# asd56585452/IGS

Hardware: AMD Instinct MI355X
Metric: Gaussians rendered/sec (fwd+bwd) at 1352x1014; PSNR vs ref (higher is better)
Workload: dtype f32; 1 GPU; BASELINE.json configs[2]: sear_steak-like frame-0 stand-in, 200000 Gaussians, SH degree 3, 10 train cams @1352x1014; per step and rank one view: fwd + L1 loss + bwd + Adam; scene=bench, points=200000, width=1352, height=1014, views=10, loss=l1, clamp=False, parallelism=one GPU: the whole step inside igs_refine_step, no exchange

## Files before the change

igs_amd/csrc/geom_bwd.hip:

```cpp
#include "geom_math.h"
#include "../../include/igs_rast.h"

__constant__ float BSH_C0 = 0.28209479177387814f;
__constant__ float BSH_C1 = 0.4886025119029199f;
__constant__ float BSH_C2[5] = { 1.0925484305920792f, -1.0925484305920792f, 0.31539156525252005f, -1.0925484305920792f,
                                 0.5462742152960396f };
__constant__ float BSH_C3[7] = { -0.5900435899266435f, 2.890611442640554f, -0.4570457994644658f, 0.3731763325901154f,
                                 -0.4570457994644658f, 1.445305721320277f, -0.5900435899266435f };

__device__ __forceinline__ float3 dnormvdv(float3 v, float3 dv) {
    const float sum2 = v.x * v.x + v.y * v.y + v.z * v.z;
    const float invsum32 = 1.0f / sqrtf(sum2 * sum2 * sum2);
    float3 r;
    r.x = ((+sum2 - v.x * v.x) * dv.x - v.y * v.x * dv.y - v.z * v.x * dv.z) * invsum32;
    r.y = (-v.x * v.y * dv.x + (sum2 - v.y * v.y) * dv.y - v.z * v.y * dv.z) * invsum32;
    r.z = (-v.x * v.z * dv.x - v.y * v.z * dv.y + (sum2 - v.z * v.z) * dv.z) * invsum32;
    return r;
}

__device__ __forceinline__ float3 sh_backward(int deg, int M, const float* __restrict__ sh, float3 dir_orig, uint32_t clamped,
                                              float3 dL_dcolor, float* __restrict__ dsh)
{
    const float len = sqrtf(dot3(dir_orig, dir_orig));
    const float x = dir_orig.x / len, y = dir_orig.y / len, z = dir_orig.z / len;
    const float3 g = make_float3((clamped & 1u) ? 0.f : dL_dcolor.x, (clamped & 2u) ? 0.f : dL_dcolor.y, (clamped & 4u) ? 0.f : dL_dcolor.z);
    auto L = [&](int k) { return make_float3(sh[3 * k], sh[3 * k + 1], sh[3 * k + 2]); };
    auto W = [&](int k, float b) { dsh[3 * k] = b * g.x; dsh[3 * k + 1] = b * g.y; dsh[3 * k + 2] = b * g.z; };
    float3 dx = make_float3(0, 0, 0), dy = make_float3(0, 0, 0), dz = make_float3(0, 0, 0);
    W(0, BSH_C0);
    if (deg > 0) {
        W(1, -BSH_C1 * y); W(2, BSH_C1 * z); W(3, -BSH_C1 * x);
        dx = L(3) * (-BSH_C1); dy = L(1) * (-BSH_C1); dz = L(2) * BSH_C1;
        if (deg > 1) {
            const float xx = x * x, yy = y * y, zz = z * z, xy = x * y, yz = y * z, xz = x * z;
            W(4, BSH_C2[0] * xy); W(5, BSH_C2[1] * yz); W(6, BSH_C2[2] * (2.f * zz - xx - yy)); W(7, BSH_C2[3] * xz);
            W(8, BSH_C2[4] * (xx - yy));
            dx = dx + (L(4) * (BSH_C2[0] * y) + L(6) * (BSH_C2[2] * 2.f * -x) + L(7) * (BSH_C2[3] * z) + L(8) * (BSH_C2[4] * 2.f * x));
            dy = dy + (L(4) * (BSH_C2[0] * x) + L(5) * (BSH_C2[1] * z) + L(6) * (BSH_C2[2] * 2.f * -y) + L(8) * (BSH_C2[4] * 2.f * -y));
            dz = dz + (L(5) * (BSH_C2[1] * y) + L(6) * (BSH_C2[2] * 2.f * 2.f * z) + L(7) * (BSH_C2[3] * x));
            if (deg > 2) {
                W(9, BSH_C3[0] * y * (3.f * xx - yy)); W(10, BSH_C3[1] * xy * z); W(11, BSH_C3[2] * y * (4.f * zz - xx - yy));
                W(12, BSH_C3[3] * z * (2.f * zz - 3.f * xx - 3.f * yy)); W(13, BSH_C3[4] * x * (4.f * zz - xx - yy));
                W(14, BSH_C3[5] * z * (xx - yy)); W(15, BSH_C3[6] * x * (xx - 3.f * yy));
                dx = dx + (L(9) * (BSH_C3[0] * 3.f * 2.f * xy) + L(10) * (BSH_C3[1] * yz) + L(11) * (BSH_C3[2] * -2.f * xy)
                           + L(12) * (BSH_C3[3] * -3.f * 2.f * xz) + L(13) * (BSH_C3[4] * (-3.f * xx + 4.f * zz - yy))
                           + L(14) * (BSH_C3[5] * 2.f * xz) + L(15) * (BSH_C3[6] * 3.f * (xx - yy)));
                dy = dy + (L(9) * (BSH_C3[0] * 3.f * (xx - yy)) + L(10) * (BSH_C3[1] * xz)
                           + L(11) * (BSH_C3[2] * (-3.f * yy + 4.f * zz - xx)) + L(12) * (BSH_C3[3] * -3.f * 2.f * yz)
                           + L(13) * (BSH_C3[4] * -2.f * xy) + L(14) * (BSH_C3[5] * -2.f * yz) + L(15) * (BSH_C3[6] * -3.f * 2.f * xy));
                dz = dz + (L(10) * (BSH_C3[1] * xy) + L(11) * (BSH_C3[2] * 4.f * 2.f * yz) + L(12) * (BSH_C3[3] * 3.f * (2.f * zz - xx - yy))
                           + L(13) * (BSH_C3[4] * 4.f * 2.f * xz) + L(14) * (BSH_C3[5] * (xx - yy)));
            }
        }
    }
    const int used = (deg + 1) * (deg + 1);
    for (int k = used; k < M; k++) { dsh[3 * k] = 0.f; dsh[3 * k + 1] = 0.f; dsh[3 * k + 2] = 0.f; }
    const float3 dL_ddir = make_float3(dot3(dx, g), dot3(dy, g), dot3(dz, g));
    return dnormvdv(dir_orig, dL_ddir);
}

__device__ __forceinline__ float3 sh_backward_dir_only(int deg, const float* __restrict__ sh, float3 dir_orig, uint32_t clamped, float3 dL_dcolor)
{
    const float len = sqrtf(dot3(dir_orig, dir_orig));
    const float x = dir_orig.x / len, y = dir_orig.y / len, z = dir_orig.z / len;
    const float3 g = make_float3((clamped & 1u) ? 0.f : dL_dcolor.x, (clamped & 2u) ? 0.f : dL_dcolor.y, (clamped & 4u) ? 0.f : dL_dcolor.z);
    auto L = [&](int k) { return make_float3(sh[3 * k], sh[3 * k + 1], sh[3 * k + 2]); };
    float3 dx = make_float3(0, 0, 0), dy = make_float3(0, 0, 0), dz = make_float3(0, 0, 0);
    if (deg > 0) {
        dx = L(3) * (-BSH_C1); dy = L(1) * (-BSH_C1); dz = L(2) * BSH_C1;
        if (deg > 1) {
            const float xx = x * x, yy = y * y, zz = z * z, xy = x * y, yz = y * z, xz = x * z;
            dx = dx + (L(4) * (BSH_C2[0] * y) + L(6) * (BSH_C2[2] * 2.f * -x) + L(7) * (BSH_C2[3] * z) + L(8) * (BSH_C2[4] * 2.f * x));
            dy = dy + (L(4) * (BSH_C2[0] * x) + L(5) * (BSH_C2[1] * z) + L(6) * (BSH_C2[2] * 2.f * -y) + L(8) * (BSH_C2[4] * 2.f * -y));
            dz = dz + (L(5) * (BSH_C2[1] * y) + L(6) * (BSH_C2[2] * 2.f * 2.f * z) + L(7) * (BSH_C2[3] * x));
            if (deg > 2) {
                dx = dx + (L(9) * (BSH_C3[0] * 3.f * 2.f * xy) + L(10) * (BSH_C3[1] * yz) + L(11) * (BSH_C3[2] * -2.f * xy)
                           + L(12) * (BSH_C3[3] * -3.f * 2.f * xz) + L(13) * (BSH_C3[4] * (-3.f * xx + 4.f * zz - yy))
                           + L(14) * (BSH_C3[5] * 2.f * xz) + L(15) * (BSH_C3[6] * 3.f * (xx - yy)));
                dy = dy + (L(9) * (BSH_C3[0] * 3.f * (xx - yy)) + L(10) * (BSH_C3[1] * xz)
                           + L(11) * (BSH_C3[2] * (-3.f * yy + 4.f * zz - xx)) + L(12) * (BSH_C3[3] * -3.f * 2.f * yz)
                           + L(13) * (BSH_C3[4] * -2.f * xy) + L(14) * (BSH_C3[5] * -2.f * yz) + L(15) * (BSH_C3[6] * -3.f * 2.f * xy));
                dz = dz + (L(10) * (BSH_C3[1] * xy) + L(11) * (BSH_C3[2] * 4.f * 2.f * yz) + L(12) * (BSH_C3[3] * 3.f * (2.f * zz - xx - yy))
                           + L(13) * (BSH_C3[4] * 4.f * 2.f * xz) + L(14) * (BSH_C3[5] * (xx - yy)));
            }
        }
    }
    const float3 dL_ddir = make_float3(dot3(dx, g), dot3(dy, g), dot3(dz, g));
    return dnormvdv(dir_orig, dL_ddir);
}

struct ShViewCams { float pos[3 * IGS_MAX_EXCHANGE_VIEWS]; };
struct ShAdam { float *param, *exp_avg, *exp_avg_sq; float lr_over_bc1, b1, b2, eps, inv_sqrt_bc2;
                float *sm_param = nullptr, *sm_exp_avg = nullptr, *sm_exp_avg_sq = nullptr; const float* sm_grad = nullptr;
                size_t sm_off[4] = {0, 0, 0, 0}; float sm_lr_over_bc1[4] = {0, 0, 0, 0}; };
template <bool ADAM>
__global__ void __launch_bounds__(128)
sh_grad_views_kernel(int P, int D, int M, int V, const float* __restrict__ means3D, const ShViewCams cams,
                     const float* __restrict__ gc, float clamp, float* __restrict__ dsh_out, const ShAdam ad)
{
    const float* campos = cams.pos;
    const int idx = blockIdx.x * 128 + threadIdx.x;
    const bool live = idx < P;
    if (!ADAM && !live) return;
    float acc[48];
#pragma unroll
    for (int k = 0; k < 48; k++) acc[k] = 0.f;
    const size_t ci = live ? (size_t)idx : 0;
    const float3 mean = make_float3(means3D[3 * ci], means3D[3 * ci + 1], means3D[3 * ci + 2]);
    for (int v = 0; v < (live ? V : 0); v++) {
        const float* gp = gc + ((size_t)v * P + idx) * 3;
        const float3 g = make_float3(gp[0], gp[1], gp[2]);
        if (g.x == 0.f && g.y == 0.f && g.z == 0.f) continue;
// ... 76 lines not shown
            for (int gk = 0; gk < 4; gk++) {
                const size_t o = ad.sm_off[gk] + (size_t)idx * KS[gk];
#pragma unroll
                for (int c = 0; c < KS[gk]; c++) {
                    float pp = ad.sm_param[o + c], mm = ad.sm_exp_avg[o + c], vv = ad.sm_exp_avg_sq[o + c];
                    adam_update(pp, mm, vv, ad.sm_grad[o + c], ad.sm_lr_over_bc1[gk], ad.b1, ad.b2, ad.eps, ad.inv_sqrt_bc2);
                    ad.sm_param[o + c] = pp; ad.sm_exp_avg[o + c] = mm; ad.sm_exp_avg_sq[o + c] = vv;
                }
            }
        }
        return;
    }
    float* dst = dsh_out + (size_t)idx * M * 3;
    if (M == 16 && (((uintptr_t)dsh_out) & 15) == 0) {
#pragma unroll
        for (int k = 0; k < 12; k++) ((float4*)dst)[k] = make_float4(acc[4 * k], acc[4 * k + 1], acc[4 * k + 2], acc[4 * k + 3]);
        return;
    }
#pragma unroll
    for (int k = 0; k < 16; k++)
        if (k < M) { dst[3 * k] = acc[3 * k]; dst[3 * k + 1] = acc[3 * k + 1]; dst[3 * k + 2] = acc[3 * k + 2]; }
}

hipError_t launch_sh_grad_views(hipStream_t s, int P, int D, int M, int V, const float* means3D, const float* campos_host, const float* gc,
                                float clamp, float* dsh_out)
{
    ShViewCams cams;
    for (int i = 0; i < 3 * V; i++) cams.pos[i] = campos_host[i];
    hipLaunchKernelGGL(sh_grad_views_kernel<false>, dim3((P + 127) / 128), dim3(128), 0, s, P, D, M, V, means3D, cams, gc, clamp, dsh_out, ShAdam());
    return hipGetLastError();
}

hipError_t launch_sh_adam_views(hipStream_t s, int P, int D, int M, int V, const float* means3D, const float* campos_host, const float* gc,
                                float clamp, float* param_sh, float* exp_avg_sh, float* exp_avg_sq_sh, float lr_over_bc1, float b1, float b2,
                                float eps, float inv_sqrt_bc2, const SmallGroupsAdam* sm)
{
    ShViewCams cams;
    for (int i = 0; i < 3 * V; i++) cams.pos[i] = campos_host[i];
    ShAdam ad; ad.param = param_sh; ad.exp_avg = exp_avg_sh; ad.exp_avg_sq = exp_avg_sq_sh;
    ad.lr_over_bc1 = lr_over_bc1; ad.b1 = b1; ad.b2 = b2; ad.eps = eps; ad.inv_sqrt_bc2 = inv_sqrt_bc2;
    if (sm) {
        ad.sm_param = sm->param; ad.sm_exp_avg = sm->exp_avg; ad.sm_exp_avg_sq = sm->exp_avg_sq; ad.sm_grad = sm->grad;
        for (int k = 0; k < 4; k++) { ad.sm_off[k] = sm->off[k]; ad.sm_lr_over_bc1[k] = sm->lr_over_bc1[k]; }
    }
    hipLaunchKernelGGL(sh_grad_views_kernel<true>, dim3((P + 127) / 128), dim3(128), 0, s, P, D, M, V, means3D, cams, gc, clamp, (float*)nullptr, ad);
    return hipGetLastError();
}

struct GBArgs { GeomBwdArgs a; RefineFuse f; };

#ifndef GEOM_WAVES_PER_EU
#define GEOM_WAVES_PER_EU 2
#endif
#ifdef GEOM_TIMELINE
#define GEOM_TL_MARKS 8
#define GEOM_TL_WGS 8192
__device__ unsigned long long g_geom_tl[GEOM_TL_WGS * GEOM_TL_MARKS];
extern "C" int igs_debug_geom_timeline(unsigned long long* host, int n)
{
    return (int)hipMemcpyFromSymbol(host, HIP_SYMBOL(g_geom_tl), (size_t)n * 8);
}
#define GTL(k) do { if (threadIdx.x == 0 && blockIdx.x < GEOM_TL_WGS) g_geom_tl[blockIdx.x * GEOM_TL_MARKS + (k)] = wall_clock64(); } while (0)
#else
#define GTL(k) do { } while (0)
#endif
template <bool FUSED, int NT, bool COLOUR_ONLY, bool PARTIAL = false>
__global__ void __launch_bounds__(NT) __attribute__((amdgpu_waves_per_eu(GEOM_WAVES_PER_EU)))
geom_bwd_kernel(const GBArgs args)
{
    const GeomBwdArgs& a = args.a;
    const RefineFuse& fz = args.f;
    if constexpr (FUSED) {
        if ((fz.guard_overflow && *fz.guard_overflow) || (fz.guard_prefilter && *fz.guard_prefilter)) return;
        if (blockIdx.x == 0 && threadIdx.x < 64 && fz.loss_out) {
            float v = fz.loss_scale * fz.loss_shards[16 * threadIdx.x];
            if (fz.loss_shards2) v += fz.loss_scale2 * fz.loss_shards2[16 * threadIdx.x];
            if (fz.loss_shards3) v += fz.loss_scale3 * fz.loss_shards3[16 * threadIdx.x];
#pragma unroll
            for (int off = 32; off > 0; off >>= 1) v += __shfl_down(v, off, 64);
            if (threadIdx.x == 0) fz.loss_out[0] = fz.loss_bias + v;
        }
    }
    GTL(0);
    const int ngroups = (a.P + NT - 1) / NT;
    for (int grp = blockIdx.x; grp < ngroups; grp += gridDim.x) {
    const int idx = grp * NT + threadIdx.x;
    extern __shared__ __attribute__((aligned(16))) float dsh_lds[];
    const int F = 3 * a.M, FS = F + 1;
    const bool active = idx < a.P;

    float3 o_m2d = make_float3(0, 0, 0), o_color = make_float3(0, 0, 0), o_mean = make_float3(0, 0, 0), o_scale = make_float3(0, 0, 0);
    float o_opacity = 0.f, o_cov[6] = { 0, 0, 0, 0, 0, 0 };
    float4 o_rot = make_float4(0, 0, 0, 0);
    const bool sh_frozen = PARTIAL && FUSED && (fz.frozen_groups & IGS_GROUP_SH) != 0u;
    float* dsh = (a.M && !sh_frozen) ? dsh_lds + threadIdx.x * FS : nullptr;
    bool sh_written = false;
    bool found_nan = false;
    __shared__ float small_lds[FUSED ? NT * 12 : 1];

    if (active && a.radii[idx] > 0) {
        const float4* R4 = (const float4*)(a.rec + (size_t)idx * REC_F);
        const double2* G2 = (const double2*)(a.gacc + (size_t)idx * ((COLOUR_ONLY || a.gacc_compact) ? GACC_COMPACT_F : GACC_F));
        auto G4 = [&](int k) { const double2 u = G2[2 * k], v = G2[2 * k + 1]; return make_float4((float)u.x, (float)u.y, (float)v.x, (float)v.y); };
        const float4 r0 = R4[0], r1 = R4[1], r2 = R4[2], r4 = R4[4], r5 = R4[5], r6 = R4[6], r7 = R4[7];
        PlaneCacheEntry pce; pce.have = false;
        if (!COLOUR_ONLY && a.plane_cache) pce = plane_cache_fetch(a.plane_cache + (size_t)idx * PLANE_CACHE_F);
        float4 g0, g1, g2, g3, g4, g5, g6;
        if (COLOUR_ONLY || a.gacc_compact) {
            const float4 c0 = G4(0), c1 = G4(1), c2 = G4(2);
            const float4 z = make_float4(0.f, 0.f, 0.f, 0.f);
            g0 = make_float4(c0.x, c0.y, c0.z, 0.f); g1 = z; g2 = z; g3 = z;
            g4 = make_float4(0.f, 0.f, c0.w, c1.x); g5 = make_float4(c1.y, c1.z, c1.w, c2.x); g6 = make_float4(c2.y, 0.f, 0.f, 0.f);
        } else {
            g0 = G4(0); g1 = G4(1); g2 = G4(2); g3 = G4(3); g4 = G4(4); g5 = G4(5); g6 = G4(6);
        }
        GTL(1);
        o_color = make_float3(g0.x, g0.y, g0.z);
        const float Sv0 = g0.w, Sv1 = g1.x, Sv2 = g1.y;
        const float Sx0 = g1.z, Sx1 = g1.w, Sx2 = g2.x, Sy0 = g2.y, Sy1 = g2.z, Sy2 = g2.w;
        const float St = g3.x, Stx = g3.y, Sty = g3.z;
        const float3 dL_dnormal = make_float3(g3.w, g4.x, g4.y);
        const float Q0 = g4.z, Qx = g4.w, Qy = g5.x, Qxx = g5.y, Qxy = g5.z, Qyy = g5.w, Z = g6.x;
        const float conx = r0.z, cony = r0.w, conz = r1.x, opac = r1.y;
        const float cpl[6] = { r4.x, r4.y, r4.z, r4.w, r5.x, r5.y };
        const float rplx = r2.z, rply = r2.w;
        const float halfW = 0.5f * a.W, halfH = 0.5f * a.H;
        o_m2d.x = (-(conx * Qx + cony * Qy) + cpl[0] * Sv0 + cpl[2] * Sv1 + cpl[4] * Sv2 + rplx * St) * halfW;
        o_m2d.y = (-(conz * Qy + cony * Qx) + cpl[1] * Sv0 + cpl[3] * Sv1 + cpl[5] * Sv2 + rply * St) * halfH;
        o_m2d.z = Z;
        const float dLc_x = -0.5f * Qxx, dLc_y = -0.5f * Qxy, dLc_z = -0.5f * Qyy;
        const float c0x = Sx0 / a.fx, c0y = Sy0 / a.fy, c1x = Sx1 / a.fx, c1y = Sy1 / a.fy, c2x = Sx2 / a.fx, c2y = Sy2 / a.fy;
        const float drx = Stx / a.fx, dry = Sty / a.fy;
        const float dL_dts = St;
        float dL_dopacity = (opac != 0.f) ? Q0 / opac : 0.f;

        const float3 mean = make_float3(a.means3D[3 * idx], a.means3D[3 * idx + 1], a.means3D[3 * idx + 2]);
        float cov3D[6];
        if (a.cov3D_precomp) {
#pragma unroll
            for (int k = 0; k < 6; k++) cov3D[k] = a.cov3D_precomp[6 * (size_t)idx + k];
        } else { cov3D[0] = r6.x; cov3D[1] = r6.y; cov3D[2] = r6.z; cov3D[3] = r6.w; cov3D[4] = r7.x; cov3D[5] = r7.y; }
        const uint32_t clamped = __float_as_uint(r7.z);

        const bool need_planes = !COLOUR_ONLY && ((Sv0 != 0.f) | (Sv1 != 0.f) | (Sv2 != 0.f) | (Sx0 != 0.f) | (Sx1 != 0.f) | (Sx2 != 0.f)
                                 | (Sy0 != 0.f) | (Sy1 != 0.f) | (Sy2 != 0.f) | (St != 0.f) | (Stx != 0.f) | (Sty != 0.f)
                                 | (dL_dnormal.x != 0.f) | (dL_dnormal.y != 0.f) | (dL_dnormal.z != 0.f));
        Cov2DCtx c;
        cov2d_ctx(c, mean, cov3D, a.view, a.fx, a.fy, a.tan_fovx, a.tan_fovy, a.kernel_size, need_planes,
// ... 196 lines not shown
                }
            }
        }
        if (a.scales) {
            float3 sc = make_float3(a.scales[3 * idx], a.scales[3 * idx + 1], a.scales[3 * idx + 2]);
            float4 qr = make_float4(a.rotations[4 * idx], a.rotations[4 * idx + 1], a.rotations[4 * idx + 2], a.rotations[4 * idx + 3]);
            if constexpr (FUSED) {
                sc = make_float3(act_exp(sc.x), act_exp(sc.y), act_exp(sc.z));
                const float inv = act_inv_norm4(qr.x, qr.y, qr.z, qr.w);
                qr = make_float4(qr.x * inv, qr.y * inv, qr.z * inv, qr.w * inv);
            }
            const float r = qr.x, x = qr.y, y = qr.z, z = qr.w;
            const M3 Rq = quat_rot(qr);
            const float s[3] = { a.scale_modifier * sc.x, a.scale_modifier * sc.y, a.scale_modifier * sc.z };
            float dS[3][3];
            dS[0][0] = o_cov[0]; dS[0][1] = 0.5f * o_cov[1]; dS[0][2] = 0.5f * o_cov[2];
            dS[1][0] = 0.5f * o_cov[1]; dS[1][1] = o_cov[3]; dS[1][2] = 0.5f * o_cov[4];
            dS[2][0] = 0.5f * o_cov[2]; dS[2][1] = 0.5f * o_cov[4]; dS[2][2] = o_cov[5];
            float dM[3][3];
#pragma unroll
            for (int k = 0; k < 3; k++)
#pragma unroll
                for (int b = 0; b < 3; b++)
                    dM[k][b] = (2.0f * (s[k] * Rq.m[0][k])) * dS[0][b] + (2.0f * (s[k] * Rq.m[1][k])) * dS[1][b] + (2.0f * (s[k] * Rq.m[2][k])) * dS[2][b];
            const float ds0 = Rq.m[0][0] * dM[0][0] + Rq.m[1][0] * dM[0][1] + Rq.m[2][0] * dM[0][2];
            const float ds1 = Rq.m[0][1] * dM[1][0] + Rq.m[1][1] * dM[1][1] + Rq.m[2][1] * dM[1][2];
            const float ds2 = Rq.m[0][2] * dM[2][0] + Rq.m[1][2] * dM[2][1] + Rq.m[2][2] * dM[2][2];
            o_scale = make_float3(ds0, ds1, ds2);
#define X_(a_, b_) (dM[a_][b_] * s[a_])
            o_rot.x = 2 * z * (X_(0, 1) - X_(1, 0)) + 2 * y * (X_(2, 0) - X_(0, 2)) + 2 * x * (X_(1, 2) - X_(2, 1));
            o_rot.y = 2 * y * (X_(1, 0) + X_(0, 1)) + 2 * z * (X_(2, 0) + X_(0, 2)) + 2 * r * (X_(1, 2) - X_(2, 1)) - 4 * x * (X_(2, 2) + X_(1, 1));
            o_rot.z = 2 * x * (X_(1, 0) + X_(0, 1)) + 2 * r * (X_(2, 0) - X_(0, 2)) + 2 * z * (X_(1, 2) + X_(2, 1)) - 4 * y * (X_(2, 2) + X_(0, 0));
            o_rot.w = 2 * r * (X_(0, 1) - X_(1, 0)) + 2 * x * (X_(2, 0) + X_(0, 2)) + 2 * y * (X_(1, 2) + X_(2, 1)) - 4 * z * (X_(1, 1) + X_(0, 0));
#undef X_
        }
    }
    if constexpr (FUSED) {
        if (active && fz.color_out && !sh_written) {
            fz.color_out[3 * (size_t)idx] = 0.f; fz.color_out[3 * (size_t)idx + 1] = 0.f; fz.color_out[3 * (size_t)idx + 2] = 0.f;
        }
    }
    if (active) {
        if (!FUSED || a.dL_dmean2D) {
            a.dL_dmean2D[3 * idx] = o_m2d.x; a.dL_dmean2D[3 * idx + 1] = o_m2d.y; a.dL_dmean2D[3 * idx + 2] = o_m2d.z;
        }
        if constexpr (!FUSED) {
            if (a.clamp > 0.f) {
                const float c = a.clamp;
                auto cl = [c](float x) { return x < -c ? -c : (x > c ? c : x); };
                o_mean = make_float3(cl(o_mean.x), cl(o_mean.y), cl(o_mean.z));
                o_opacity = cl(o_opacity);
                o_scale = make_float3(cl(o_scale.x), cl(o_scale.y), cl(o_scale.z));
                o_rot = make_float4(cl(o_rot.x), cl(o_rot.y), cl(o_rot.z), cl(o_rot.w));
                if (dsh && sh_written) for (int k = 0; k < F; k++) dsh[k] = cl(dsh[k]);
            }
            a.dL_dcolor[3 * idx] = o_color.x; a.dL_dcolor[3 * idx + 1] = o_color.y; a.dL_dcolor[3 * idx + 2] = o_color.z;
            a.dL_dopacity[idx] = o_opacity;
            a.dL_dmean3D[3 * idx] = o_mean.x; a.dL_dmean3D[3 * idx + 1] = o_mean.y; a.dL_dmean3D[3 * idx + 2] = o_mean.z;
#pragma unroll
            for (int k = 0; k < 6; k++) a.dL_dcov3D[6 * (size_t)idx + k] = o_cov[k];
            a.dL_dscale[3 * idx] = o_scale.x; a.dL_dscale[3 * idx + 1] = o_scale.y; a.dL_dscale[3 * idx + 2] = o_scale.z;
            a.dL_drot[4 * idx] = o_rot.x; a.dL_drot[4 * idx + 1] = o_rot.y; a.dL_drot[4 * idx + 2] = o_rot.z; a.dL_drot[4 * idx + 3] = o_rot.w;
            if (a.nan_host) {
                const float chk[17] = { o_m2d.x, o_m2d.y, o_m2d.z, o_color.x, o_color.y, o_color.z, o_opacity, o_mean.x, o_mean.y, o_mean.z,
                                        o_scale.x, o_scale.y, o_scale.z, o_rot.x, o_rot.y, o_rot.z, o_rot.w };
#pragma unroll
                for (int k = 0; k < 17; k++) found_nan |= chk[k] != chk[k];
            }
        } else {
            if (fz.clamp > 0.f) {
                const float c = fz.clamp;
                auto cl = [c](float x) { return x < -c ? -c : (x > c ? c : x); };
                o_mean = make_float3(cl(o_mean.x), cl(o_mean.y), cl(o_mean.z));
                o_opacity = cl(o_opacity);
                o_scale = make_float3(cl(o_scale.x), cl(o_scale.y), cl(o_scale.z));
                o_rot = make_float4(cl(o_rot.x), cl(o_rot.y), cl(o_rot.z), cl(o_rot.w));
                if (dsh && sh_written) for (int k = 0; k < F; k++) dsh[k] = cl(dsh[k]);
            }
            const float g_xyz[3] = { o_mean.x, o_mean.y, o_mean.z };
            const float s_op = act_sigmoid(fz.param[fz.off_opacity + idx]);
            const float g_logit = o_opacity * s_op * (1.0f - s_op);
            float g_ls[3], g_rot[4];
            {
                const float* ls = fz.param + fz.off_scale + 3 * (size_t)idx;
                const float go[3] = { o_scale.x, o_scale.y, o_scale.z };
#pragma unroll
                for (int k = 0; k < 3; k++) g_ls[k] = go[k] * act_exp(ls[k]);
                const float* rq = fz.param + fz.off_rot + 4 * (size_t)idx;
                const float q0 = rq[0], q1 = rq[1], q2 = rq[2], q3 = rq[3];
                const float len = sqrtf(q0 * q0 + q1 * q1 + q2 * q2 + q3 * q3);
                const float nrm = fmaxf(len, 1e-12f);
                const float inv = 1.0f / nrm;
                const float n0 = q0 * inv, n1 = q1 * inv, n2 = q2 * inv, n3 = q3 * inv;
                const float dt = n0 * o_rot.x + n1 * o_rot.y + n2 * o_rot.z + n3 * o_rot.w;
                g_rot[0] = (o_rot.x - n0 * dt) * inv; g_rot[1] = (o_rot.y - n1 * dt) * inv;
                g_rot[2] = (o_rot.z - n2 * dt) * inv; g_rot[3] = (o_rot.w - n3 * dt) * inv;
                if (len < 1e-12f) {
                    g_rot[0] = o_rot.x * inv; g_rot[1] = o_rot.y * inv; g_rot[2] = o_rot.z * inv; g_rot[3] = o_rot.w * inv;
                }
            }
            float* sg = small_lds + threadIdx.x * 12;
            sg[0] = g_xyz[0]; sg[1] = g_xyz[1]; sg[2] = g_xyz[2];
            sg[3] = g_rot[0]; sg[4] = g_rot[1]; sg[5] = g_rot[2]; sg[6] = g_rot[3];
            sg[7] = g_logit; sg[8] = g_ls[0]; sg[9] = g_ls[1]; sg[10] = g_ls[2];
        }
        if (dsh && !sh_written) for (int k = 0; k < F; k++) dsh[k] = 0.f;
    }
    GTL(3);
    if (a.M) {
        __syncthreads();
        const int g0 = grp * NT;
        const int ng = min(NT, a.P - g0);
        bool fast_done = false;
        if constexpr (FUSED) {
            const size_t bx = fz.off_xyz + (size_t)g0 * 3, br = fz.off_rot + (size_t)g0 * 4, bo = fz.off_opacity + (size_t)g0,
                         bs = fz.off_scale + (size_t)g0 * 3, bh = fz.off_sh + (size_t)g0 * F;
            const uintptr_t pa = (uintptr_t)fz.param, ma = (uintptr_t)fz.exp_avg, va = (uintptr_t)fz.exp_avg_sq;
            const bool al = !fz.grad_out && ((F & 3) == 0) && (((pa | ma | va) & 15) == 0) && (((bx | br | bo | bs | bh) & 3) == 0)
                            && ((ng & 3) == 0);
            if (al) {
                fast_done = true;
                auto adam4 = [&](float4& P4, float4& M4, float4& V4, float g0_, float g1_, float g2_, float g3_, float lr) {
                    adam_update(P4.x, M4.x, V4.x, g0_, lr, fz.b1, fz.b2, fz.eps, fz.inv_sqrt_bc2);
                    adam_update(P4.y, M4.y, V4.y, g1_, lr, fz.b1, fz.b2, fz.eps, fz.inv_sqrt_bc2);
                    adam_update(P4.z, M4.z, V4.z, g2_, lr, fz.b1, fz.b2, fz.eps, fz.inv_sqrt_bc2);
                    adam_update(P4.w, M4.w, V4.w, g3_, lr, fz.b1, fz.b2, fz.eps, fz.inv_sqrt_bc2);
                };
                const size_t sb[4] = { bx, br, bo, bs };
                const int sk[4] = { 3, 4, 1, 3 }, sfirst[4] = { 0, 3, 7, 8 };
                const float slr[4] = { fz.lr_xyz, fz.lr_rot, fz.lr_opacity, fz.lr_scale };
                float4 SP[4], SM[4], SV[4];
                const bool qlive[4] = { true, true, !PARTIAL || (fz.frozen_groups & IGS_GROUP_OPACITY) == 0u, !PARTIAL || (fz.frozen_groups & IGS_GROUP_SCALE) == 0u };
#pragma unroll
                for (int q = 0; q < 4; q++) {
                    const bool ok = qlive[q] && (int)threadIdx.x < (ng * sk[q]) / 4;
                    const size_t o = sb[q] / 4 + threadIdx.x;
                    if (ok) { SP[q] = ((const float4*)fz.param)[o]; SM[q] = ld_moment((const float4*)fz.exp_avg + o); SV[q] = ld_moment((const float4*)fz.exp_avg_sq + o); }
                }
                const int total4 = sh_frozen ? 0 : (ng * F) >> 2;
                constexpr int UB = 2;
                float4 HP[UB], HM[UB], HV[UB];
                auto sh_load = [&](int batch) {
#pragma unroll
                    for (int u = 0; u < UB; u++) {
                        const int i = (int)threadIdx.x + (batch * UB + u) * NT;
                        if (i < total4) {
                            const size_t o = bh / 4 + i;
                            HP[u] = ((const float4*)fz.param)[o]; HM[u] = ld_moment((const float4*)fz.exp_avg + o); HV[u] = ld_moment((const float4*)fz.exp_avg_sq + o);
                        }
                    }
                };
                int row_g = (4 * (int)threadIdx.x) / F, row_k = 4 * (int)threadIdx.x - row_g * F;
                const int row_dg = (4 * NT) / F, row_dk = 4 * NT - row_dg * F;
                auto sh_finish = [&](int batch) {
#pragma unroll
                    for (int u = 0; u < UB; u++) {
                        const int i = (int)threadIdx.x + (batch * UB + u) * NT;
                        if (i < total4) {
                            const float* sp = dsh_lds + row_g * FS + row_k;
                            adam4(HP[u], HM[u], HV[u], sp[0], sp[1], sp[2], sp[3], fz.lr_sh);
                            const size_t o = bh / 4 + i;
                            st_param((float4*)fz.param + o, HP[u]); st_moment((float4*)fz.exp_avg + o, HM[u]); st_moment((float4*)fz.exp_avg_sq + o, HV[u]);
                        }
                        row_g += row_dg; row_k += row_dk;
                        if (row_k >= F) { row_k -= F; row_g++; }
                    }
                };
                const int nbatch = (total4 + UB * NT - 1) / (UB * NT);
                if (nbatch > 0) sh_load(0);
#pragma unroll
                for (int q = 0; q < 4; q++) {
                    if (qlive[q] && (int)threadIdx.x < (ng * sk[q]) / 4) {
                        float g[4];
#pragma unroll
                        for (int c = 0; c < 4; c++) { const int e = 4 * (int)threadIdx.x + c, gl = e / sk[q]; g[c] = small_lds[gl * 12 + sfirst[q] + (e - gl * sk[q])]; }
                        adam4(SP[q], SM[q], SV[q], g[0], g[1], g[2], g[3], slr[q]);
                        const size_t o = sb[q] / 4 + threadIdx.x;
                        st_param((float4*)fz.param + o, SP[q]); st_moment((float4*)fz.exp_avg + o, SM[q]); st_moment((float4*)fz.exp_avg_sq + o, SV[q]);
                    }
                }
                GTL(4);
                for (int b = 0; b < nbatch; b++) {
                    sh_finish(b);
                    if (b + 1 < nbatch) sh_load(b + 1);
                }
            }
        }
        if (!fast_done) {
        if constexpr (FUSED) {
            auto small_group = [&](size_t off, int k, int first, float lr) {
                const size_t base = off + (size_t)g0 * k;
                const int n = ng * k;
                float* P = fz.grad_out ? fz.grad_out + base : fz.param + base;
                float* Mo = fz.exp_avg + base; float* Vo = fz.exp_avg_sq + base;
                const bool al = (((uintptr_t)P | (uintptr_t)Mo | (uintptr_t)Vo) & 15) == 0;
                const int n4 = al ? n >> 2 : 0;
                for (int i = threadIdx.x; i < n4; i += NT) {
                    float g[4];
#pragma unroll
                    for (int q = 0; q < 4; q++) { const int e = 4 * i + q, gl = e / k; g[q] = small_lds[gl * 12 + first + (e - gl * k)]; }
                    if (fz.grad_out) { ((float4*)P)[i] = make_float4(g[0], g[1], g[2], g[3]); continue; }
                    float4 P4 = ((float4*)P)[i], M4 = ((float4*)Mo)[i], V4 = ((float4*)Vo)[i];
                    adam_update(P4.x, M4.x, V4.x, g[0], lr, fz.b1, fz.b2, fz.eps, fz.inv_sqrt_bc2);
                    adam_update(P4.y, M4.y, V4.y, g[1], lr, fz.b1, fz.b2, fz.eps, fz.inv_sqrt_bc2);
                    adam_update(P4.z, M4.z, V4.z, g[2], lr, fz.b1, fz.b2, fz.eps, fz.inv_sqrt_bc2);
                    adam_update(P4.w, M4.w, V4.w, g[3], lr, fz.b1, fz.b2, fz.eps, fz.inv_sqrt_bc2);
                    ((float4*)P)[i] = P4; ((float4*)Mo)[i] = M4; ((float4*)Vo)[i] = V4;
                }
                for (int e = 4 * n4 + threadIdx.x; e < n; e += NT) {
                    const int gl = e / k;
                    const float g = small_lds[gl * 12 + first + (e - gl * k)];
                    if (fz.grad_out) { P[e] = g; continue; }
                    float p = P[e], m = Mo[e], v = Vo[e];
                    adam_update(p, m, v, g, lr, fz.b1, fz.b2, fz.eps, fz.inv_sqrt_bc2);
                    P[e] = p; Mo[e] = m; Vo[e] = v;
                }
            };
            small_group(fz.off_xyz, 3, 0, fz.lr_xyz);
            small_group(fz.off_rot, 4, 3, fz.lr_rot);
            if (!PARTIAL || !(fz.frozen_groups & IGS_GROUP_OPACITY)) small_group(fz.off_opacity, 1, 7, fz.lr_opacity);
            if (!PARTIAL || !(fz.frozen_groups & IGS_GROUP_SCALE)) small_group(fz.off_scale, 3, 8, fz.lr_scale);
        }
        const bool skip_sh = sh_frozen || (FUSED && fz.grad_out && (fz.color_out || fz.colors_extracted));
        if (!skip_sh) {
        const int total = ng * F;
        float* dst = FUSED ? fz.param + fz.off_sh + (size_t)g0 * F : a.dL_dsh + (size_t)g0 * F;
        float* dst_m = FUSED ? fz.exp_avg + fz.off_sh + (size_t)g0 * F : nullptr;
        float* dst_v = FUSED ? fz.exp_avg_sq + fz.off_sh + (size_t)g0 * F : nullptr;
        bool aligned = ((F & 3) == 0) && ((((uintptr_t)dst) & 15) == 0);
        if constexpr (FUSED) aligned = aligned && (((((uintptr_t)dst_m) | ((uintptr_t)dst_v)) & 15) == 0)
                                       && (!fz.grad_out || (((uintptr_t)(fz.grad_out + fz.off_sh + (size_t)g0 * F)) & 15) == 0);
        if (aligned) {
            const int total4 = total >> 2;
            int f = (int)threadIdx.x * 4;
            int g = f / F, k = f - g * F;
            const int dg = (4 * NT) / F, dk = (4 * NT) - dg * F;
            for (int i = threadIdx.x; i < total4; i += NT) {
                const float* sp = dsh_lds + g * FS + k;
                if (FUSED && fz.grad_out) {
                    ((float4*)(fz.grad_out + fz.off_sh + (size_t)g0 * F))[i] = make_float4(sp[0], sp[1], sp[2], sp[3]);
                } else if constexpr (FUSED) {
                    float4 P4 = ((float4*)dst)[i], M4 = ((float4*)dst_m)[i], V4 = ((float4*)dst_v)[i];
                    adam_update(P4.x, M4.x, V4.x, sp[0], fz.lr_sh, fz.b1, fz.b2, fz.eps, fz.inv_sqrt_bc2);
                    adam_update(P4.y, M4.y, V4.y, sp[1], fz.lr_sh, fz.b1, fz.b2, fz.eps, fz.inv_sqrt_bc2);
                    adam_update(P4.z, M4.z, V4.z, sp[2], fz.lr_sh, fz.b1, fz.b2, fz.eps, fz.inv_sqrt_bc2);
                    adam_update(P4.w, M4.w, V4.w, sp[3], fz.lr_sh, fz.b1, fz.b2, fz.eps, fz.inv_sqrt_bc2);
                    ((float4*)dst)[i] = P4; ((float4*)dst_m)[i] = M4; ((float4*)dst_v)[i] = V4;
                } else {
                    ((float4*)dst)[i] = make_float4(sp[0], sp[1], sp[2], sp[3]);
                    if (a.nan_host) found_nan |= (sp[0] != sp[0]) | (sp[1] != sp[1]) | (sp[2] != sp[2]) | (sp[3] != sp[3]);
                }
                g += dg; k += dk;
                if (k >= F) { k -= F; g++; }
            }
        } else {
            int f = (int)threadIdx.x;
            int g = f / F, k = f - g * F;
            const int dg = NT / F, dk = NT - dg * F;
            for (int i = threadIdx.x; i < total; i += NT) {
                if (FUSED && fz.grad_out) {
                    fz.grad_out[fz.off_sh + (size_t)g0 * F + i] = dsh_lds[g * FS + k];
                } else if constexpr (FUSED) {
                    float p = dst[i], m = dst_m[i], v = dst_v[i];
                    adam_update(p, m, v, dsh_lds[g * FS + k], fz.lr_sh, fz.b1, fz.b2, fz.eps, fz.inv_sqrt_bc2);
                    dst[i] = p; dst_m[i] = m; dst_v[i] = v;
                } else {
                    dst[i] = dsh_lds[g * FS + k];
                    if (a.nan_host) found_nan |= dst[i] != dst[i];
                }
                g += dg; k += dk;
                if (k >= F) { k -= F; g++; }
            }
        }
        }
        }
    }
    GTL(5);
    if constexpr (!FUSED) {
        if (a.nan_host && found_nan) __atomic_store_n(a.nan_host, a.nan_seq, __ATOMIC_RELAXED);
    }
    if (grp + (int)gridDim.x < ngroups) __syncthreads();
    }
}

hipError_t launch_geom_bwd(hipStream_t s, const GeomBwdArgs& a)
{
    GBArgs g; g.a = a; g.f = RefineFuse();
    const size_t lds = a.M ? (size_t)256 * (3 * a.M + 1) * sizeof(float) : 0;
    hipLaunchKernelGGL((geom_bwd_kernel<false, 256, false>), dim3((a.P + 255) / 256), dim3(256), lds, s, g);
    return hipGetLastError();
}
#ifndef GEOM_ADAM_THREADS
#define GEOM_ADAM_THREADS 64
#endif
#ifndef GEOM_ADAM_BLOCKS
#define GEOM_ADAM_BLOCKS (1 << 30)
#endif
hipError_t launch_geom_bwd_adam(hipStream_t s, const GeomBwdArgs& a, const RefineFuse& f)
{
    GBArgs g; g.a = a; g.f = f;
    if (f.first > 0) {
        const size_t F0 = (size_t)f.first;
        if (f.first > a.P || f.grad_out || f.color_out || a.dL_dmean2D) return hipErrorInvalidValue;
        g.a.P = a.P - f.first;
        g.a.radii = a.radii + F0; g.a.rec = a.rec + F0 * REC_F;
        g.a.means3D = a.means3D + 3 * F0; g.a.scales = a.scales ? a.scales + 3 * F0 : nullptr;
        g.a.rotations = a.rotations ? a.rotations + 4 * F0 : nullptr; g.a.shs = a.shs ? a.shs + F0 * 3 * a.M : nullptr;
        if (a.plane_cache) g.a.plane_cache = a.plane_cache + F0 * PLANE_CACHE_F;
        if (a.cov3D_precomp) g.a.cov3D_precomp = a.cov3D_precomp + 6 * F0;
        g.f.off_xyz += 3 * F0; g.f.off_rot += 4 * F0; g.f.off_sh += F0 * 3 * a.M; g.f.off_opacity += F0; g.f.off_scale += 3 * F0;
    }
    constexpr int NT = GEOM_ADAM_THREADS;
    const size_t lds = (a.M && !(f.frozen_groups & IGS_GROUP_SH)) ? (size_t)NT * (3 * a.M + 1) * sizeof(float) : 0;
    int blocks = (g.a.P + NT - 1) / NT;
    if (blocks < 1) blocks = 1;
    const int cap = GEOM_ADAM_BLOCKS;
    if (blocks > cap) blocks = cap;
    if (f.frozen_groups) {
        if (a.gacc_compact) hipLaunchKernelGGL((geom_bwd_kernel<true, NT, true, true>), dim3(blocks), dim3(NT), lds, s, g);
        else                hipLaunchKernelGGL((geom_bwd_kernel<true, NT, false, true>), dim3(blocks), dim3(NT), lds, s, g);
    } else if (a.gacc_compact) hipLaunchKernelGGL((geom_bwd_kernel<true, NT, true>), dim3(blocks), dim3(NT), lds, s, g);
    else                       hipLaunchKernelGGL((geom_bwd_kernel<true, NT, false>), dim3(blocks), dim3(NT), lds, s, g);
    return hipGetLastError();
}

__global__ void __launch_bounds__(256)
extract_view_colors_kernel(int P, const int* __restrict__ radii, const float* __restrict__ rec, const double* __restrict__ gacc,
                           int stride, int have_sh, float* __restrict__ color_out)
{
    const int idx = blockIdx.x * 256 + threadIdx.x;
    if (idx >= P) return;
    float3 c = make_float3(0.f, 0.f, 0.f);
    if (have_sh && radii[idx] > 0) {
        const double* gr = gacc + (size_t)idx * stride;
        const float3 g = make_float3((float)gr[0], (float)gr[1], (float)gr[2]);
        const uint32_t clamped = __float_as_uint(rec[(size_t)idx * REC_F + 30]);
        c = make_float3((clamped & 1u) ? 0.f : g.x, (clamped & 2u) ? 0.f : g.y, (clamped & 4u) ? 0.f : g.z);
    }
    color_out[3 * (size_t)idx] = c.x; color_out[3 * (size_t)idx + 1] = c.y; color_out[3 * (size_t)idx + 2] = c.z;
}
hipError_t launch_extract_view_colors(hipStream_t s, int P, const int* radii, const float* rec, const double* gacc, int gacc_compact, bool have_sh,
                                      float* color_out)
{
    hipLaunchKernelGGL(extract_view_colors_kernel, dim3((P + 255) / 256), dim3(256), 0, s, P, radii, rec, gacc,
                       gacc_compact ? GACC_COMPACT_F : GACC_F, have_sh ? 1 : 0, color_out);
    return hipGetLastError();
}
```

Measured before the change: 829.1 million Gaussians/s.

## Store SH basis and colour gradient in LDS instead of full dSH

```diff
diff --git a/igs_amd/csrc/geom_bwd.hip b/igs_amd/csrc/geom_bwd.hip
--- a/igs_amd/csrc/geom_bwd.hip
+++ b/igs_amd/csrc/geom_bwd.hip
@@ -19,13 +19,14 @@
 }
 
 __device__ __forceinline__ float3 sh_backward(int deg, int M, const float* __restrict__ sh, float3 dir_orig, uint32_t clamped,
-                                              float3 dL_dcolor, float* __restrict__ dsh)
+                                              float3 dL_dcolor, float* __restrict__ bas)
 {
     const float len = sqrtf(dot3(dir_orig, dir_orig));
     const float x = dir_orig.x / len, y = dir_orig.y / len, z = dir_orig.z / len;
     const float3 g = make_float3((clamped & 1u) ? 0.f : dL_dcolor.x, (clamped & 2u) ? 0.f : dL_dcolor.y, (clamped & 4u) ? 0.f : dL_dcolor.z);
     auto L = [&](int k) { return make_float3(sh[3 * k], sh[3 * k + 1], sh[3 * k + 2]); };
-    auto W = [&](int k, float b) { dsh[3 * k] = b * g.x; dsh[3 * k + 1] = b * g.y; dsh[3 * k + 2] = b * g.z; };
+    auto W = [&](int k, float b) { bas[k] = b; };
+    bas[M] = g.x; bas[M + 1] = g.y; bas[M + 2] = g.z;
     float3 dx = make_float3(0, 0, 0), dy = make_float3(0, 0, 0), dz = make_float3(0, 0, 0);
     W(0, BSH_C0);
     if (deg > 0) {
@@ -53,11 +54,45 @@
             }
         }
     }
-    const int used = (deg + 1) * (deg + 1);
-    for (int k = used; k < M; k++) { dsh[3 * k] = 0.f; dsh[3 * k + 1] = 0.f; dsh[3 * k + 2] = 0.f; }
     const float3 dL_ddir = make_float3(dot3(dx, g), dot3(dy, g), dot3(dz, g));
     return dnormvdv(dir_orig, dL_ddir);
 }
+
+__device__ __forceinline__ float sh_grad1(const float* bas, int M, int used, int kr, int kc, float clamp)
+{
+    float x = kr < used ? bas[kr] * bas[M + kc] : 0.f;
+    if (clamp > 0.f) x = x < -clamp ? -clamp : (x > clamp ? clamp : x);
+    return x;
+}
+__device__ __forceinline__ float4 sh_grad4(const float* bas, int M, int used, int kr, int kc, float clamp)
+{
+    float v[4];
+#pragma unroll
+    for (int j = 0; j < 4; j++) {
+        v[j] = sh_grad1(bas, M, used, kr, kc, clamp);
+        if (++kc == 3) { kc = 0; kr++; }
+    }
+    return make_float4(v[0], v[1], v[2], v[3]);
+}
+__device__ __forceinline__ void adam_update_sh(float& p, float& m, float& v, float g, float lr, float b1, float b2, float eps, float inv_sqrt_bc2)
+{
+#pragma clang fp contract(off)
+    m = __builtin_fmaf(b1, m, (1.f - b1) * g);
+    v = __builtin_fmaf(b2, v, (1.f - b2) * g * g);
+    p -= lr * m / __builtin_fmaf(sqrtf(v), inv_sqrt_bc2, eps);
+}
+struct ShCursor {
+    int gl, kr, kc, dg, dkr, dkc;
+    __device__ __forceinline__ ShCursor(int e0, int step, int M) {
+        const int F = 3 * M;
+        gl = e0 / F; const int k = e0 - gl * F; kr = k / 3; kc = k - 3 * kr;
+        dg = step / F; const int dk = step - dg * F; dkr = dk / 3; dkc = dk - 3 * dkr;
+    }
+    __device__ __forceinline__ void next(int M) {
+        kc += dkc; if (kc >= 3) { kc -= 3; kr++; }
+        kr += dkr; gl += dg; if (kr >= M) { kr -= M; gl++; }
+    }
+};
 
 __device__ __forceinline__ float3 sh_backward_dir_only(int deg, const float* __restrict__ sh, float3 dir_orig, uint32_t clamped, float3 dL_dcolor)
 {
@@ -240,6 +275,9 @@
 #ifndef GEOM_WAVES_PER_EU
 #define GEOM_WAVES_PER_EU 2
 #endif
+#ifndef GEOM_WAVES_PER_EU_COLOUR
+#define GEOM_WAVES_PER_EU_COLOUR 4
+#endif
 #ifdef GEOM_TIMELINE
 #define GEOM_TL_MARKS 8
 #define GEOM_TL_WGS 8192
@@ -253,7 +291,7 @@
 #define GTL(k) do { } while (0)
 #endif
 template <bool FUSED, int NT, bool COLOUR_ONLY, bool PARTIAL = false>
-__global__ void __launch_bounds__(NT) __attribute__((amdgpu_waves_per_eu(GEOM_WAVES_PER_EU)))
+__global__ void __launch_bounds__(NT) __attribute__((amdgpu_waves_per_eu(COLOUR_ONLY ? GEOM_WAVES_PER_EU_COLOUR : GEOM_WAVES_PER_EU)))
 geom_bwd_kernel(const GBArgs args)
 {
     const GeomBwdArgs& a = args.a;
@@ -270,18 +308,19 @@
         }
     }
     GTL(0);
-    const int ngroups = (a.P + NT - 1) / NT;
-    for (int grp = blockIdx.x; grp < ngroups; grp += gridDim.x) {
+    const int grp = blockIdx.x;
     const int idx = grp * NT + threadIdx.x;
-    extern __shared__ __attribute__((aligned(16))) float dsh_lds[];
-    const int F = 3 * a.M, FS = F + 1;
+    extern __shared__ __attribute__((aligned(16))) float sh_lds[];
+    const int F = 3 * a.M, SS = a.M + 4;
+    const int sh_used = min((a.D + 1) * (a.D + 1), a.M);
+    const float sh_clamp = FUSED ? fz.clamp : a.clamp;
     const bool active = idx < a.P;
 
     float3 o_m2d = make_float3(0, 0, 0), o_color = make_float3(0, 0, 0), o_mean = make_float3(0, 0, 0), o_scale = make_float3(0, 0, 0);
     float o_opacity = 0.f, o_cov[6] = { 0, 0, 0, 0, 0, 0 };
     float4 o_rot = make_float4(0, 0, 0, 0);
     const bool sh_frozen = PARTIAL && FUSED && (fz.frozen_groups & IGS_GROUP_SH) != 0u;
-    float* dsh = (a.M && !sh_frozen) ? dsh_lds + threadIdx.x * FS : nullptr;
+    float* dsh = (a.M && !sh_frozen) ? sh_lds + threadIdx.x * SS : nullptr;
     bool sh_written = false;
     bool found_nan = false;
     __shared__ float small_lds[FUSED ? NT * 12 : 1];
@@ -584,7 +623,6 @@
                 o_opacity = cl(o_opacity);
                 o_scale = make_float3(cl(o_scale.x), cl(o_scale.y), cl(o_scale.z));
                 o_rot = make_float4(cl(o_rot.x), cl(o_rot.y), cl(o_rot.z), cl(o_rot.w));
-                if (dsh && sh_written) for (int k = 0; k < F; k++) dsh[k] = cl(dsh[k]);
             }
             a.dL_dcolor[3 * idx] = o_color.x; a.dL_dcolor[3 * idx + 1] = o_color.y; a.dL_dcolor[3 * idx + 2] = o_color.z;
             a.dL_dopacity[idx] = o_opacity;
@@ -607,7 +645,6 @@
                 o_opacity = cl(o_opacity);
                 o_scale = make_float3(cl(o_scale.x), cl(o_scale.y), cl(o_scale.z));
                 o_rot = make_float4(cl(o_rot.x), cl(o_rot.y), cl(o_rot.z), cl(o_rot.w));
-                if (dsh && sh_written) for (int k = 0; k < F; k++) dsh[k] = cl(dsh[k]);
             }
             const float g_xyz[3] = { o_mean.x, o_mean.y, o_mean.z };
             const float s_op = act_sigmoid(fz.param[fz.off_opacity + idx]);
@@ -636,7 +673,7 @@
             sg[3] = g_rot[0]; sg[4] = g_rot[1]; sg[5] = g_rot[2]; sg[6] = g_rot[3];
             sg[7] = g_logit; sg[8] = g_ls[0]; sg[9] = g_ls[1]; sg[10] = g_ls[2];
         }
-        if (dsh && !sh_written) for (int k = 0; k < F; k++) dsh[k] = 0.f;
+        if (dsh && !sh_written) for (int k = 0; k < a.M + 3; k++) dsh[k] = 0.f;
     }
     GTL(3);
     if (a.M) {
@@ -652,69 +689,57 @@
                             && ((ng & 3) == 0);
             if (al) {
                 fast_done = true;
-                auto adam4 = [&](float4& P4, float4& M4, float4& V4, float g0_, float g1_, float g2_, float g3_, float lr) {
-                    adam_update(P4.x, M4.x, V4.x, g0_, lr, fz.b1, fz.b2, fz.eps, fz.inv_sqrt_bc2);
-                    adam_update(P4.y, M4.y, V4.y, g1_, lr, fz.b1, fz.b2, fz.eps, fz.inv_sqrt_bc2);
-                    adam_update(P4.z, M4.z, V4.z, g2_, lr, fz.b1, fz.b2, fz.eps, fz.inv_sqrt_bc2);
-                    adam_update(P4.w, M4.w, V4.w, g3_, lr, fz.b1, fz.b2, fz.eps, fz.inv_sqrt_bc2);
+                constexpr int UB = 2;
+                float4 HP[UB], HM[UB], HV[UB];
+                auto load = [&](int u, size_t o) {
+                    HP[u] = ((const float4*)fz.param)[o]; HM[u] = ld_moment((const float4*)fz.exp_avg + o); HV[u] = ld_moment((const float4*)fz.exp_avg_sq + o);
+                };
+                auto store = [&](int u, size_t o) {
+                    st_param((float4*)fz.param + o, HP[u]); st_moment((float4*)fz.exp_avg + o, HM[u]); st_moment((float4*)fz.exp_avg_sq + o, HV[u]);
                 };
                 const size_t sb[4] = { bx, br, bo, bs };
                 const int sk[4] = { 3, 4, 1, 3 }, sfirst[4] = { 0, 3, 7, 8 };
                 const float slr[4] = { fz.lr_xyz, fz.lr_rot, fz.lr_opacity, fz.lr_scale };
-                float4 SP[4], SM[4], SV[4];
                 const bool qlive[4] = { true, true, !PARTIAL || (fz.frozen_groups & IGS_GROUP_OPACITY) == 0u, !PARTIAL || (fz.frozen_groups & IGS_GROUP_SCALE) == 0u };
 #pragma unroll
-                for (int q = 0; q < 4; q++) {
-                    const bool ok = qlive[q] && (int)threadIdx.x < (ng * sk[q]) / 4;
-                    const size_t o = sb[q] / 4 + threadIdx.x;
-                    if (ok) { SP[q] = ((const float4*)fz.param)[o]; SM[q] = ld_moment((const float4*)fz.exp_avg + o); SV[q] = ld_moment((const float4*)fz.exp_avg_sq + o); }
-                }
-                const int total4 = sh_frozen ? 0 : (ng * F) >> 2;
-                constexpr int UB = 2;
-                float4 HP[UB], HM[UB], HV[UB];
-                auto sh_load = [&](int batch) {
+                for (int q0 = 0; q0 < 4; q0 += UB) {
+#pragma unroll
+                    for (int u = 0; u < UB; u++)
+                        if (qlive[q0 + u] && (int)threadIdx.x < (ng * sk[q0 + u]) / 4) load(u, sb[q0 + u] / 4 + threadIdx.x);
 #pragma unroll
                     for (int u = 0; u < UB; u++) {
-                        const int i = (int)threadIdx.x + (batch * UB + u) * NT;
-                        if (i < total4) {
-                            const size_t o = bh / 4 + i;
-                            HP[u] = ((const float4*)fz.param)[o]; HM[u] = ld_moment((const float4*)fz.exp_avg + o); HV[u] = ld_moment((const float4*)fz.exp_avg_sq + o);
+                        const int q = q0 + u;
+                        if (qlive[q] && (int)threadIdx.x < (ng * sk[q]) / 4) {
+                            float g[4];
+#pragma unroll
+                            for (int c = 0; c < 4; c++) { const int e = 4 * (int)threadIdx.x + c, gl = e / sk[q]; g[c] = small_lds[gl * 12 + sfirst[q] + (e - gl * sk[q])]; }
+                            adam_update(HP[u].x, HM[u].x, HV[u].x, g[0], slr[q], fz.b1, fz.b2, fz.eps, fz.inv_sqrt_bc2);
+                            adam_update(HP[u].y, HM[u].y, HV[u].y, g[1], slr[q], fz.b1, fz.b2, fz.eps, fz.inv_sqrt_bc2);
+                            adam_update(HP[u].z, HM[u].z, HV[u].z, g[2], slr[q], fz.b1, fz.b2, fz.eps, fz.inv_sqrt_bc2);
+                            adam_update(HP[u].w, HM[u].w, HV[u].w, g[3], slr[q], fz.b1, fz.b2, fz.eps, fz.inv_sqrt_bc2);
+                            store(u, sb[q] / 4 + threadIdx.x);
                         }
                     }
-                };
-                int row_g = (4 * (int)threadIdx.x) / F, row_k = 4 * (int)threadIdx.x - row_g * F;
-                const int row_dg = (4 * NT) / F, row_dk = 4 * NT - row_dg * F;
-                auto sh_finish = [&](int batch) {
+                }
+                GTL(4);
+                const int total4 = sh_frozen ? 0 : (ng * F) >> 2;
+                ShCursor cur(4 * (int)threadIdx.x, 4 * NT, a.M);
+                for (int i0 = threadIdx.x; i0 < total4; i0 += UB * NT) {
+#pragma unroll
+                    for (int u = 0; u < UB; u++)
+                        if (i0 + u * NT < total4) load(u, bh / 4 + i0 + u * NT);
 #pragma unroll
                     for (int u = 0; u < UB; u++) {
-                        const int i = (int)threadIdx.x + (batch * UB + u) * NT;
-                        if (i < total4) {
-                            const float* sp = dsh_lds + row_g * FS + row_k;
-                            adam4(HP[u], HM[u], HV[u], sp[0], sp[1], sp[2], sp[3], fz.lr_sh);
-                            const size_t o = bh / 4 + i;
-                            st_param((float4*)fz.param + o, HP[u]); st_moment((float4*)fz.exp_avg + o, HM[u]); st_moment((float4*)fz.exp_avg_sq + o, HV[u]);
+                        if (i0 + u * NT < total4) {
+                            const float4 g = sh_grad4(sh_lds + cur.gl * SS, a.M, sh_used, cur.kr, cur.kc, sh_clamp);
+                            adam_update_sh(HP[u].x, HM[u].x, HV[u].x, g.x, fz.lr_sh, fz.b1, fz.b2, fz.eps, fz.inv_sqrt_bc2);
+                            adam_update_sh(HP[u].y, HM[u].y, HV[u].y, g.y, fz.lr_sh, fz.b1, fz.b2, fz.eps, fz.inv_sqrt_bc2);
+                            adam_update_sh(HP[u].z, HM[u].z, HV[u].z, g.z, fz.lr_sh, fz.b1, fz.b2, fz.eps, fz.inv_sqrt_bc2);
+                            adam_update_sh(HP[u].w, HM[u].w, HV[u].w, g.w, fz.lr_sh, fz.b1, fz.b2, fz.eps, fz.inv_sqrt_bc2);
+                            store(u, bh / 4 + i0 + u * NT);
                         }
-                        row_g += row_dg; row_k += row_dk;
-                        if (row_k >= F) { row_k -= F; row_g++; }
+                        cur.next(a.M);
                     }
-                };
-                const int nbatch = (total4 + UB * NT - 1) / (UB * NT);
-                if (nbatch > 0) sh_load(0);
-#pragma unroll
-                for (int q = 0; q < 4; q++) {
-                    if (qlive[q] && (int)threadIdx.x < (ng * sk[q]) / 4) {
-                        float g[4];
-#pragma unroll
-                        for (int c = 0; c < 4; c++) { const int e = 4 * (int)threadIdx.x + c, gl = e / sk[q]; g[c] = small_lds[gl * 12 + sfirst[q] + (e - gl * sk[q])]; }
-                        adam4(SP[q], SM[q], SV[q], g[0], g[1], g[2], g[3], slr[q]);
-                        const size_t o = sb[q] / 4 + threadIdx.x;
-                        st_param((float4*)fz.param + o, SP[q]); st_moment((float4*)fz.exp_avg + o, SM[q]); st_moment((float4*)fz.exp_avg_sq + o, SV[q]);
-                    }
-                }
-                GTL(4);
-                for (int b = 0; b < nbatch; b++) {
-                    sh_finish(b);
-                    if (b + 1 < nbatch) sh_load(b + 1);
                 }
             }
         }
@@ -764,44 +789,37 @@
                                        && (!fz.grad_out || (((uintptr_t)(fz.grad_out + fz.off_sh + (size_t)g0 * F)) & 15) == 0);
         if (aligned) {
             const int total4 = total >> 2;
-            int f = (int)threadIdx.x * 4;
-            int g = f / F, k = f - g * F;
-            const int dg = (4 * NT) / F, dk = (4 * NT) - dg * F;
-            for (int i = threadIdx.x; i < total4; i += NT) {
-                const float* sp = dsh_lds + g * FS + k;
+            ShCursor cur(4 * (int)threadIdx.x, 4 * NT, a.M);
+            for (int i = threadIdx.x; i < total4; i += NT, cur.next(a.M)) {
+                const float4 sp = sh_grad4(sh_lds + cur.gl * SS, a.M, sh_used, cur.kr, cur.kc, sh_clamp);
                 if (FUSED && fz.grad_out) {
-                    ((float4*)(fz.grad_out + fz.off_sh + (size_t)g0 * F))[i] = make_float4(sp[0], sp[1], sp[2], sp[3]);
+                    ((float4*)(fz.grad_out + fz.off_sh + (size_t)g0 * F))[i] = sp;
                 } else if constexpr (FUSED) {
                     float4 P4 = ((float4*)dst)[i], M4 = ((float4*)dst_m)[i], V4 = ((float4*)dst_v)[i];
-                    adam_update(P4.x, M4.x, V4.x, sp[0], fz.lr_sh, fz.b1, fz.b2, fz.eps, fz.inv_sqrt_bc2);
-                    adam_update(P4.y, M4.y, V4.y, sp[1], fz.lr_sh, fz.b1, fz.b2, fz.eps, fz.inv_sqrt_bc2);
-                    adam_update(P4.z, M4.z, V4.z, sp[2], fz.lr_sh, fz.b1, fz.b2, fz.eps, fz.inv_sqrt_bc2);
-                    adam_update(P4.w, M4.w, V4.w, sp[3], fz.lr_sh, fz.b1, fz.b2, fz.eps, fz.inv_sqrt_bc2);
+                    adam_update_sh(P4.x, M4.x, V4.x, sp.x, fz.lr_sh, fz.b1, fz.b2, fz.eps, fz.inv_sqrt_bc2);
+                    adam_update_sh(P4.y, M4.y, V4.y, sp.y, fz.lr_sh, fz.b1, fz.b2, fz.eps, fz.inv_sqrt_bc2);
+                    adam_update_sh(P4.z, M4.z, V4.z, sp.z, fz.lr_sh, fz.b1, fz.b2, fz.eps, fz.inv_sqrt_bc2);
+                    adam_update_sh(P4.w, M4.w, V4.w, sp.w, fz.lr_sh, fz.b1, fz.b2, fz.eps, fz.inv_sqrt_bc2);
                     ((float4*)dst)[i] = P4; ((float4*)dst_m)[i] = M4; ((float4*)dst_v)[i] = V4;
                 } else {
-                    ((float4*)dst)[i] = make_float4(sp[0], sp[1], sp[2], sp[3]);
-                    if (a.nan_host) found_nan |= (sp[0] != sp[0]) | (sp[1] != sp[1]) | (sp[2] != sp[2]) | (sp[3] != sp[3]);
-                }
-                g += dg; k += dk;
-                if (k >= F) { k -= F; g++; }
+                    ((float4*)dst)[i] = sp;
+                    if (a.nan_host) found_nan |= (sp.x != sp.x) | (sp.y != sp.y) | (sp.z != sp.z) | (sp.w != sp.w);
+                }
             }
         } else {
-            int f = (int)threadIdx.x;
-            int g = f / F, k = f - g * F;
-            const int dg = NT / F, dk = NT - dg * F;
-            for (int i = threadIdx.x; i < total; i += NT) {
+            ShCursor cur((int)threadIdx.x, NT, a.M);
+            for (int i = threadIdx.x; i < total; i += NT, cur.next(a.M)) {
+                const float gv = sh_grad1(sh_lds + cur.gl * SS, a.M, sh_used, cur.kr, cur.kc, sh_clamp);
                 if (FUSED && fz.grad_out) {
-                    fz.grad_out[fz.off_sh + (size_t)g0 * F + i] = dsh_lds[g * FS + k];
+                    fz.grad_out[fz.off_sh + (size_t)g0 * F + i] = gv;
                 } else if constexpr (FUSED) {
                     float p = dst[i], m = dst_m[i], v = dst_v[i];
-                    adam_update(p, m, v, dsh_lds[g * FS + k], fz.lr_sh, fz.b1, fz.b2, fz.eps, fz.inv_sqrt_bc2);
+                    adam_update_sh(p, m, v, gv, fz.lr_sh, fz.b1, fz.b2, fz.eps, fz.inv_sqrt_bc2);
                     dst[i] = p; dst_m[i] = m; dst_v[i] = v;
                 } else {
-                    dst[i] = dsh_lds[g * FS + k];
-                    if (a.nan_host) found_nan |= dst[i] != dst[i];
-                }
-                g += dg; k += dk;
-                if (k >= F) { k -= F; g++; }
+                    dst[i] = gv;
+                    if (a.nan_host) found_nan |= gv != gv;
+                }
             }
         }
         }
@@ -811,23 +829,19 @@
     if constexpr (!FUSED) {
         if (a.nan_host && found_nan) __atomic_store_n(a.nan_host, a.nan_seq, __ATOMIC_RELAXED);
     }
-    if (grp + (int)gridDim.x < ngroups) __syncthreads();
-    }
 }
 
 hipError_t launch_geom_bwd(hipStream_t s, const GeomBwdArgs& a)
 {
     GBArgs g; g.a = a; g.f = RefineFuse();
-    const size_t lds = a.M ? (size_t)256 * (3 * a.M + 1) * sizeof(float) : 0;
+    const size_t lds = a.M ? (size_t)256 * (a.M + 4) * sizeof(float) : 0;
     hipLaunchKernelGGL((geom_bwd_kernel<false, 256, false>), dim3((a.P + 255) / 256), dim3(256), lds, s, g);
     return hipGetLastError();
 }
 #ifndef GEOM_ADAM_THREADS
 #define GEOM_ADAM_THREADS 64
 #endif
-#ifndef GEOM_ADAM_BLOCKS
-#define GEOM_ADAM_BLOCKS (1 << 30)
-#endif
+extern "C" size_t igs_geom_bwd_adam_dyn_lds(int M) { return (size_t)GEOM_ADAM_THREADS * (M + 4) * sizeof(float); }
 hipError_t launch_geom_bwd_adam(hipStream_t s, const GeomBwdArgs& a, const RefineFuse& f)
 {
     GBArgs g; g.a = a; g.f = f;
@@ -843,11 +857,9 @@
         g.f.off_xyz += 3 * F0; g.f.off_rot += 4 * F0; g.f.off_sh += F0 * 3 * a.M; g.f.off_opacity += F0; g.f.off_scale += 3 * F0;
     }
     constexpr int NT = GEOM_ADAM_THREADS;
-    const size_t lds = (a.M && !(f.frozen_groups & IGS_GROUP_SH)) ? (size_t)NT * (3 * a.M + 1) * sizeof(float) : 0;
+    const size_t lds = (a.M && !(f.frozen_groups & IGS_GROUP_SH)) ? igs_geom_bwd_adam_dyn_lds(a.M) : 0;
     int blocks = (g.a.P + NT - 1) / NT;
     if (blocks < 1) blocks = 1;
-    const int cap = GEOM_ADAM_BLOCKS;
-    if (blocks > cap) blocks = cap;
     if (f.frozen_groups) {
         if (a.gacc_compact) hipLaunchKernelGGL((geom_bwd_kernel<true, NT, true, true>), dim3(blocks), dim3(NT), lds, s, g);
         else                hipLaunchKernelGGL((geom_bwd_kernel<true, NT, false, true>), dim3(blocks), dim3(NT), lds, s, g);
```

Measured after the change: 863.7 million Gaussians/s, median of 6. +4.2%, better.
